# magenta/music-spectrogram-diffusion

Hardware: AMD Instinct MI355X
Metric: mel-frames/sec (higher is better)
Workload: dtype f16x3 (operands split into hi + lo half planes, 3 f16 MFMAs per product, fp32 accumulate; fp32 residual/norm/softmax/sampler); 1 GPU; base_with_context, 1000-step DDPM, CFG w=5, 1 song(s) per GPU, segment-sequential with context hand-off, 5 segments of 256 frames per GPU; precision=f16x3, precision_requested=f16x3, parallelism=song-parallel x1, mode=replicas, attention_query_planes=library default: hi + lo for Q and for the softmax weights, knobs=library defaults

## Files before the change

### include/msd_amd.h

```cpp
#ifndef MSD_AMD_H_
#define MSD_AMD_H_

#include <stdint.h>

#ifdef __cplusplus
extern "C" {
#endif

#define MSD_AMD_ABI_VERSION 7

typedef struct msd_model msd_model;

typedef enum msd_status {
  MSD_OK = 0,
  MSD_ERR_INVALID_ARGUMENT = 1,
  MSD_ERR_UNKNOWN_WEIGHT = 2,
  MSD_ERR_SHAPE_MISMATCH = 3,
  MSD_ERR_BAD_STATE = 4,
  MSD_ERR_HIP = 5,
  MSD_ERR_UNSUPPORTED = 6,
  MSD_ERR_RANGE = 7
} msd_status;

typedef enum msd_precision {
// ... 147 lines not shown
                              const float* w1_dev, const float* gamma_dev,
                              const float* film_scale_dev, const float* film_bias_dev,
                              const float* w2_dev, float* x_out_dev, float* h_out_dev,
                              int m, int k, int d, int n, void* stream);

int msd_op_geglu(const float* a_dev, const float* wi0_dev, const float* wi1_dev, float* out_dev,
                 int m, int k, int f, void* stream);

int msd_op_qkv(const float* a_dev, const float* wq_dev, const float* wk_dev, const float* wv_dev,
               float* q_out_dev, float* k_out_dev, float* v_out_dev, int m, int k, int j,
               int seg_len, void* stream);

int msd_op_final_proj(const float* x_dev, const float* gamma_dev, const float* w_dev, float* out_dev,
                      int m, int d, int n, void* stream);

int msd_op_threefry(int stage, uint64_t seed, int64_t fold, const uint32_t* bits_in_dev, float* out_dev, int64_t n,
                    void* stream);

#ifdef __cplusplus
}
#endif
#endif
```

### music-spectrogram-diffusion_amd/build_native.py

```python
from __future__ import annotations

import os
import shutil
import subprocess
import sys

HERE = os.path.dirname(os.path.abspath(__file__))
ROOT = os.path.dirname(HERE)
CSRC = os.path.join(HERE, 'csrc')
EXP = os.path.join(ROOT, 'tools', 'ubench', 'exp')
LIB = os.path.join(CSRC, 'libmsd_amd.so')
LIB_EXP = os.path.join(EXP, 'libmsd_amd_exp.so')
LIBS = {'f16': (LIB, []), 'bf16': (os.path.join(CSRC, 'libmsd_amd_bf16.so'), ['-DMSD_PLANE_BF16=1'])}
EXP_SRC = os.path.join(EXP, 'src_r04')
EXP_LIBS = {'exp': (LIB_EXP, ['-DMSD_EXPERIMENTS=1'])}
SOURCES = ['msd_api.hip']
HEADERS = ['common.h', 'phase_stamps.h', 'gemm_h16.h', 'gemm_f32.h', 'attention.h', 'elementwise.h',
           os.path.join('..', '..', 'include', 'msd_amd.h')]
EXP_HEADERS = ['chain.h', 'gemm_h16_exp.h', 'gemm_splitk_exchange.inc', 'gemm_h16_pair.h', 'gemm_h16_wide.h', 'gemm_h16_ls.h']


def _hipcc():
  for c in (os.environ.get('HIPCC'), shutil.which('hipcc'), '/opt/rocm/bin/hipcc'):
    if c and os.path.exists(c):
# ... 11 lines not shown
    deps = [os.path.join(CSRC, f) for f in SOURCES + HEADERS + [os.path.join('..', 'build_native.py')]]
  return any(os.path.getmtime(f) > t for f in deps)


def check_prefetch_registers(listing: str) -> str:
  tool = os.path.join(HERE, 'check_prefetch_regs.py')
  if not os.path.exists(tool):
    raise RuntimeError('%s is missing: the build cannot verify the prefetch registers of the library' % tool)
  out = subprocess.run([sys.executable, tool, listing], capture_output=True, text=True)
  if out.returncode != 0:
    raise RuntimeError('prefetch register check failed on %s:\n%s\n%s' % (listing, out.stdout[-3000:], out.stderr[-2000:]))
  return out.stdout.strip().split('\n')[-1]


NO_SCRATCH_KERNELS = ('sampler_step_kernel', 'threefry_normal_kernel')


def check_no_scratch(listing: str, kernels=NO_SCRATCH_KERNELS) -> str:
  import re
  text = open(listing).read()
  seen = {k: 0 for k in kernels}
  bad = []
  for m in re.finditer(r'^\s*\.amdhsa_kernel\s+(\S+)(.*?)^\s*\.end_amdhsa_kernel', text, flags=re.M | re.S):
    name, body = m.group(1), m.group(2)
    for k in kernels:
      if k in name:
        seen[k] += 1
        size = re.search(r'\.amdhsa_private_segment_fixed_size\s+(\d+)', body)
        dyn = re.search(r'\.amdhsa_uses_dynamic_stack\s+(\d+)', body)
        if size is None or int(size.group(1)) != 0 or (dyn is not None and int(dyn.group(1)) != 0):
# ... 22 lines not shown
             '-fno-gpu-rdc', '-Wno-unused-result', '-ffile-prefix-map=%s=.' % ROOT, '-ffile-prefix-map=%s=.' % tmp,
             '-cuid=msd_amd',
             '-I', src] + defs + ['-o', os.path.basename(lib)] + [os.path.join(src, s) for s in SOURCES]
      if verbose:
        print('[build_native]', ' '.join(cmd), flush=True)
      subprocess.run(cmd, check=True, cwd=tmp)
      listings = [os.path.join(tmp, f) for f in os.listdir(tmp) if f.endswith('.s') and 'gfx950' in f]
      if not listings:
        raise RuntimeError('no gfx950 device listing (*gfx950*.s, -save-temps) in %s: cannot verify the prefetch '
                           'registers; the scratch directory holds %s' % (tmp, sorted(os.listdir(tmp))))
      for l in listings:
        verdict = check_prefetch_registers(l)
        if verbose:
          print('[build_native] prefetch registers:', verdict, flush=True)
        if src == CSRC:
          verdict = check_no_scratch(l)
          if verbose:
            print('[build_native] scratch:', verdict, flush=True)
      shutil.copyfile(out, lib + '.tmp')
      os.chmod(lib + '.tmp', 0o755)
      os.replace(lib + '.tmp', lib)
  return LIB


if __name__ == '__main__':
  build(force='--force' in sys.argv, experiments='--experiments' in sys.argv)
  print(LIB)
```

### music-spectrogram-diffusion_amd/csrc/elementwise.h

```cpp
#pragma once
#include "common.h"

namespace msd {

struct NormParams {
  const float* x;
  const float* gamma;
  const float* film;
  const int* step_ptr;
  int film_slots, film_slot;
  int rows, D;
  h16_t* out[2];
  float* out_f32;
  unsigned* sat = nullptr;
  unsigned sat_tag = 1;
};

template <int OUT, int VPL>
__global__ void __launch_bounds__(256) rmsnorm_film_kernel(NormParams p) {
  const int lane = threadIdx.x & 63;
  const int row = blockIdx.x * 4 + (threadIdx.x >> 6);
  if (row >= p.rows) return;
  const float* xr = p.x + (size_t)row * p.D;
  float4 v[VPL];
// ... 183 lines not shown
  const uint32_t* rng_key = nullptr;
  const float* coef;
  int* step_ptr;
  int step_from_slot1 = 0;
  int n;
  int passes;
  float cond_wt;
  int clip_x0, ddim;
  int model_output = kOutEps;
  h16_t* z_hi;
  h16_t* z_lo;
  unsigned* sat = nullptr;
  unsigned sat_tag = 1;
};

template <int mode>
__device__ __forceinline__ void convert_model_output(const float (&c)[kCoefCount], float z, float o,
                                                     float& eps, float& x0) {
  if constexpr (mode == kOutEps) {
    eps = o;
    x0 = c[kCoefMX0Scale] * (z - o * c[kCoefMX0Eps]);
  } else if constexpr (mode == kOutX0) {
    x0 = o;
    eps = c[kCoefMEpsScale] * (z - o * c[kCoefMEpsX0]);
  } else {
    x0 = c[kCoefMAlpha] * z - c[kCoefMSigma] * o;
    eps = c[kCoefMEpsScale] * (z - x0 * c[kCoefMEpsX0]);
  }
}

template <int MODE>
__device__ __forceinline__ float sampler_update(const SamplerParams& p, const float (&c)[kCoefCount], int i, float z,
                                                float o_c, float o_u, float nz) {
  float eps, x0;
  convert_model_output<MODE>(c, z, o_c, eps, x0);
  if (p.passes == 2) {
    float eps_u, x0_u;
    convert_model_output<MODE>(c, z, o_u, eps_u, x0_u);
    eps = p.cond_wt * eps + (1.0f - p.cond_wt) * eps_u;
    x0 = c[kCoefX0Scale] * (z - eps * c[kCoefX0Eps]);
  }
  if (p.clip_x0) {
    x0 = x0 < -1.0f ? -1.0f : (x0 > 1.0f ? 1.0f : x0);
    eps = c[kCoefEpsScale] * (z - x0 * c[kCoefEpsX0]);
  }
  float zs;
  if (p.ddim) zs = c[kCoefAlphaS] * x0 + c[kCoefSigmaS] * eps;
  else zs = c[kCoefMeanZ] * z + c[kCoefMeanX0] * x0 + c[kCoefStd] * nz;
  return (i == 0) ? x0 : zs;
}

template <int MODE>
__global__ void __launch_bounds__(256) sampler_step_kernel(SamplerParams p) {
  warm_kernargs<kernarg_lines<SamplerParams>()>();
  const int i = p.step_from_slot1 ? p.step_ptr[1] : p.step_ptr[0];
  typedef uint32_t u32x4 __attribute__((ext_vector_type(4)));
  const float* noise = *p.noise_slot;
  u32x4 rk0 = reinterpret_cast<const u32x4*>(p.rng_key)[0], rk1 = reinterpret_cast<const u32x4*>(p.rng_key)[1];
  static_assert(kRngKind == 4 && kRngTfKey0 == 5 && kRngTfKey1 == 6, "rk1 = {kind, Threefry key, pad}");
  asm volatile("" : "+v"(noise), "+v"(rk0), "+v"(rk1));
  const int idx = (blockIdx.x * 256 + threadIdx.x) * 4;
  if (idx < p.n) {
    const f32x4 zz = *reinterpret_cast<const f32x4*>(p.z + idx);
    const f32x4 ec = *reinterpret_cast<const f32x4*>(p.eps + idx);
    f32x4 eu = {0.f, 0.f, 0.f, 0.f}, nz = {0.f, 0.f, 0.f, 0.f};
    if (p.passes == 2) eu = *reinterpret_cast<const f32x4*>(p.eps + p.n + idx);
    static_assert(kCoefCount == 20, "five 16-byte loads per row");
    f32x4 cr[5];
#pragma unroll
    for (int k = 0; k < 5; ++k) cr[k] = reinterpret_cast<const f32x4*>(p.coef + (size_t)i * kCoefCount)[k];
    if (!p.ddim && i != 0) {
      if (noise != nullptr) {
        nz = *reinterpret_cast<const f32x4*>(noise + (size_t)i * p.n + idx);
      } else if (rk1[0] == kRngThreefry) {
        uint32_t f0 = 0u, f1 = (uint32_t)i;
        threefry2x32(rk1[1], rk1[2], f0, f1);
        const uint32_t half = (uint32_t)p.n >> 1;
#pragma unroll
        for (int k = 0; k < 4; ++k) nz[k] = threefry_normal_at(f0, f1, (uint32_t)(idx + k), half);
      } else {
        float d[4];
        philox_normal4((uint32_t)(idx >> 2), 1u + (uint32_t)i, rk0[0], rk0[1], rk0[2], rk0[3], d);
        nz = f32x4{d[0], d[1], d[2], d[3]};
      }
    }
    float c[kCoefCount];
#pragma unroll
    for (int k = 0; k < kCoefCount; ++k) c[k] = cr[k >> 2][k & 3];
    f32x4 out;
#pragma unroll
    for (int k = 0; k < 4; ++k) out[k] = sampler_update<MODE>(p, c, i, zz[k], ec[k], eu[k], nz[k]);
    *reinterpret_cast<f32x4*>(p.z + idx) = out;
    if (p.z_hi) {
      uint32_t h[2], l[2];
      RangeCheck rc;
#pragma unroll
      for (int k = 0; k < 2; ++k) {
        rc.see(out[2 * k], out[2 * k + 1]);
        split2_h16(out[2 * k], out[2 * k + 1], h[k], l[k]);
      }
      *reinterpret_cast<uint2*>(p.z_hi + idx) = make_uint2(h[0], h[1]);
      if (p.z_lo) *reinterpret_cast<uint2*>(p.z_lo + idx) = make_uint2(l[0], l[1]);
      rc.commit(p.sat, p.sat_tag);
    }
  }
  __syncthreads();
  if (blockIdx.x == gridDim.x - 1 && threadIdx.x == 0) p.step_ptr[p.step_from_slot1 ? 0 : 1] = i - 1;
}

inline void launch_sampler_step(const SamplerParams& sp, hipStream_t s) {
  const dim3 grid((sp.n / 4 + 255) / 256), block(256);
  if (sp.model_output == kOutX0) hipLaunchKernelGGL(sampler_step_kernel<kOutX0>, grid, block, 0, s, sp);
  else if (sp.model_output == kOutV) hipLaunchKernelGGL(sampler_step_kernel<kOutV>, grid, block, 0, s, sp);
  else hipLaunchKernelGGL(sampler_step_kernel<kOutEps>, grid, block, 0, s, sp);
}

__global__ void build_g_kernel(const float* film, const float* gamma, float* g, int n_steps, int slots,
                               int slot, int D) {
  const int i = blockIdx.x * 256 + threadIdx.x;
// ... 89 lines not shown
```

### music-spectrogram-diffusion_amd/csrc/gemm_f32.h

```cpp
#pragma once
#include "common.h"

namespace msd {

struct GemmF32Params {
  const float* A;
  const float* B;
  int lda, ldb;
  int M, N, K;
};

struct EpiF32Store {
  float* out;
  int ldc;
  __device__ void operator()(int m, int n, float v) const { out[(size_t)m * ldc + n] = v; }
};
struct EpiF32Swish {
  float* out;
  int ldc;
  __device__ void operator()(int m, int n, float v) const {
    out[(size_t)m * ldc + n] = v / (1.0f + expf(-v));
  }
};
struct EpiF32StoreGated {
// ... 161 lines not shown
  for (int i = 0; i < RT; ++i)
#pragma unroll
    for (int j = 0; j < 2; ++j)
#pragma unroll
      for (int e = 0; e < 4; ++e) red[wave][i * 16 + g * 4 + e][j * 16 + r] = acc[i][j][e];
  __syncthreads();
  for (int item = threadIdx.x; item < BMR * 32; item += 64 * kFinalProjWaves) {
    const int m = item >> 5, n = item & 31;
    float v = 0.f;
#pragma unroll
    for (int w = 0; w < kFinalProjWaves; ++w) v += red[w][m][n];
    p.out[(size_t)(m0 + m) * p.N + n0 + n] = v * rstd[m];
  }
}

__global__ void scale_rows_kernel(const float* w, const float* gamma, float* wg, int K, int N) {
  const int i = blockIdx.x * 256 + threadIdx.x;
  if (i < K * N) wg[i] = gamma[i / N] * w[i];
}

template <class Epi>
inline hipError_t launch_gemm_f32(const GemmF32Params& p, const Epi& epi, hipStream_t stream) {
  const int grid = ((p.M + 63) / 64) * (p.N / 64);
  hipLaunchKernelGGL(gemm_f32_kernel<Epi>, dim3(grid), dim3(256), 0, stream, p, epi);
  return hipGetLastError();
}

}
```

### music-spectrogram-diffusion_amd/csrc/msd_api.hip

```cpp
#include <hip/hip_runtime.h>
#include <algorithm>
#include <cctype>
#include <cmath>
#include <cstdarg>
#include <cstdio>
#include <cstdlib>
#include <cstring>
#include <string>
#include <unordered_map>
#include <vector>

#include "../../include/msd_amd.h"
#include "attention.h"
#include "common.h"
#include "elementwise.h"
#include "gemm_h16.h"
#include "gemm_f32.h"

using namespace msd;

namespace {

constexpr int kHeadDim = 64;
constexpr int kDefaultQPlanes = 2, kDefaultPPlanes = 2;
// ... 930 lines not shown
    return to.bn == kNarrowTile;
  }
}

template <int NP>
EpiResidualNorm<NP, false, true> with_y2(const EpiResidualNorm<NP>& e, const Planes& y2, const float* g2, int rows) {
  EpiResidualNorm<NP, false, true> o;
  o.x = e.x; o.ldx = e.ldx; o.y[0] = e.y[0]; o.y[1] = e.y[1]; o.ssq = e.ssq; o.tiles = e.tiles;
  o.g_lo = e.g_lo; o.g_lo_stride = e.g_lo_stride; o.g_hi = e.g_hi; o.g_hi_stride = e.g_hi_stride;
  o.split_row = e.split_row; o.step_ptr = e.step_ptr; o.dup_rows = e.dup_rows;
  o.y2[0] = y2.p[0]; o.y2[1] = y2.p[NP - 1]; o.g2 = g2; o.y2_rows = rows;
  return o;
}

template <int NP>
void decoder_layers(Ctx& c, int batch, int P, bool cond0, bool dedup0 = false) {
  msd_model* m = c.m;
  const int D = m->D, J = m->J, F = m->F, T = m->T;
  const int BT = batch * T, M = P * BT;
  const int slots = 2 * m->Ld, tiles = D / kNarrowTile;
  const Planes &y = m->y, &qk = m->qk, &vts = m->vt, &ao = m->ao, &gb = m->g;
  float* const x = m->x;
  float* const ssq = m->ssq;
  float* const eps = m->eps;
  const int* const nkeys_self = m->d_nkeys_self;
  auto rowscale = [&](const float* bias, int stride) {
    RowScale r;
    r.ssq = ssq; r.tiles = tiles; r.inv_d = 1.0f / (float)D; r.bias = bias; r.bias_step_stride = stride;
    r.step_ptr = m->d_step;
    return r;
  };
// ... 123 lines not shown
      const bool fold_next = !last_layer && fold_cross_q<NP>(m, batch, P, cond0, false);
      WeightPrefetch pf_qkv = last_layer ? WeightPrefetch() : prefetch_of<NP>(m, m->dec[l + 1].self.wqkv, 3 * J + (fold_next ? nq : 0), D);
      if (fold_next) {
        if constexpr (NP == 2)
          gemm<NP, TK_TALL>(c, KC_GEMM_MLP_OUT, gb, F, w.mlp.wo, F, M, D, F, with_y2<NP>(eo, m->xg, m->dec[l + 1].ln_cross, BT), 0, &pf_qkv);
      } else {
        gemm<NP, TK_TALL>(c, KC_GEMM_MLP_OUT, gb, F, w.mlp.wo, F, M, D, F, eo, 0, &pf_qkv);
      }
    }
  }
  if (NP == 2) {
    FinalProjParams fp;
    fp.x = x; fp.wg = m->w_out_g; fp.ssq = ssq; fp.out = eps;
    fp.M = M; fp.N = m->ND; fp.K = D; fp.tiles = tiles; fp.inv_d = 1.0f / (float)D;
    c.begin(KC_FINAL_PROJ);
    hipLaunchKernelGGL(final_proj_f32_kernel<1>, dim3(m->ND / 32, M / 16), dim3(64 * kFinalProjWaves), 0, c.s, fp);
    c.end(KC_FINAL_PROJ);
  } else {
    EpiStoreF32 ef;
    ef.out = eps; ef.ldc = m->ND; ef.rsc = rowscale(nullptr, 0);
    gemm<NP, TK_NARROW>(c, KC_FINAL_PROJ, y, D, m->w_out_p, D, M, m->ND, D, ef);
  }
}

template <int NP>
void in_proj(Ctx& c, int batch, int P, bool publish_step = false, bool fold0 = false) {
  msd_model* m = c.m;
  const int BT = batch * m->T;
  EpiInProj<NP> ei;
  ei.x = m->x; ei.ldx = m->D; ei.pos = m->dec_pos; ei.T = m->T; ei.pass_rows = BT; ei.passes = P;
  ei.y[0] = m->y.p[0]; ei.y[1] = m->y.p[NP - 1]; ei.ssq = m->ssq; ei.tiles = m->D / kNarrowTile;
// ... 3 lines not shown
  WeightPrefetch pf = prefetch_of<NP>(m, m->dec[0].self.wqkv, 3 * m->J + (fold0 ? m->n_cross * m->J : 0), m->D);
  gemm<NP, TK_NARROW>(c, KC_IN_PROJ, m->zp, m->ND, m->w_in_p, m->ND, BT, m->D, m->ND, ei, 0, &pf);
}

void split_z(msd_model* m, int64_t n, hipStream_t s) {
  hipLaunchKernelGGL(split_planes_kernel, dim3((unsigned)((n + 255) / 256)), dim3(256), 0, s, m->z, m->zp.p[0],
                     m->NP == 2 ? m->zp.p[1] : (h16_t*)nullptr, n, m->d_sat, (unsigned)KC_SAMPLER + 1u);
}

template <int NP>
void enqueue_step(Ctx& c, int batch) {
  msd_model* m = c.m;
  const int P = m->passes;
  const bool dedup0 = P == 2 && m->dedup_layer0;
  in_proj<NP>(c, batch, dedup0 ? 1 : P, true, fold_cross_q<NP>(m, batch, P, true, dedup0));
  decoder_layers<NP>(c, batch, P, true, dedup0);
  SamplerParams sp;
  sp.eps = m->eps; sp.z = m->z; sp.noise_slot = m->d_noise_slot; sp.coef = m->d_coef; sp.rng_key = m->d_rng_key;
  sp.step_ptr = m->d_step; sp.n = batch * m->T * m->ND; sp.passes = P;
  sp.cond_wt = m->cfg.cfg_weight; sp.clip_x0 = m->cfg.clip_x0;
  sp.ddim = m->cfg.sampler == MSD_SAMPLER_DDIM;
  sp.model_output = m->cfg.model_output;
  sp.z_hi = m->zp.p[0];
  sp.z_lo = m->NP == 2 ? m->zp.p[1] : nullptr;
  sp.sat = m->d_sat; sp.sat_tag = (unsigned)KC_SAMPLER + 1u;
  c.begin(KC_SAMPLER);
  sp.step_from_slot1 = 1;
  launch_sampler_step(sp, c.s);
  c.end(KC_SAMPLER);
}

void set_func_attrs() {
  (void)attention_prepare<1, 3>();
  (void)attention_prepare<2, 2>();
  (void)prepare_gemms<1>();
  (void)prepare_gemms<2>();
}


}

extern "C" {
// ... 958 lines not shown
  if (hipMemcpyAsync(h.data(), f32, (size_t)M * J * sizeof(float), hipMemcpyDeviceToHost, s) != hipSuccess ||
      hipStreamSynchronize(s) != hipSuccess)
    return MSD_ERR_HIP;
  for (int m = 0; m < M; ++m) {
    const int seg = m / seg_len, key = m % seg_len, o16 = key & 15;
    const int kp = (key & ~15) + 8 * ((o16 >> 2) & 1) + (o16 & 3) + 4 * (o16 >> 3);
    for (int j = 0; j < J; ++j) vh[(size_t)m * J + j] = h[((size_t)seg * J + j) * seg_len + kp];
  }
  if (hipMemcpy(q_out_dev, qh.data(), qh.size() * sizeof(float), hipMemcpyHostToDevice) != hipSuccess ||
      hipMemcpy(k_out_dev, kh.data(), kh.size() * sizeof(float), hipMemcpyHostToDevice) != hipSuccess ||
      hipMemcpy(v_out_dev, vh.data(), vh.size() * sizeof(float), hipMemcpyHostToDevice) != hipSuccess)
    return MSD_ERR_HIP;
  return MSD_OK;
}

int msd_op_final_proj(const float* x_dev, const float* gamma_dev, const float* w_dev, float* out_dev, int M, int D,
                      int n, void* stream) {
  if (M % 64 || D % 64 || n % 32 || M <= 0 || D > 1024 || !x_dev || !gamma_dev || !w_dev || !out_dev)
    return MSD_ERR_INVALID_ARGUMENT;
  hipStream_t s = static_cast<hipStream_t>(stream);
  Scratch sc;
  const int tiles = D / kNarrowTile;
  float* x = sc.get<float>((size_t)M * D);
  float* ssq = sc.get<float>((size_t)M * tiles);
  float* wg = sc.get<float>((size_t)D * n);
  int* step = sc.get<int>(2);
  Planes za, zw;
  for (int i = 0; i < 2; ++i) { za.p[i] = sc.get<h16_t>((size_t)M * 64); zw.p[i] = sc.get<h16_t>((size_t)D * 64); }
  if (!x || !ssq || !wg || !step || !za.p[1] || !zw.p[1]) return MSD_ERR_HIP;
  if (hipMemcpyAsync(x, x_dev, (size_t)M * D * sizeof(float), hipMemcpyDeviceToDevice, s) != hipSuccess) return MSD_ERR_HIP;
  EpiResidualNorm<2> er;
  er.x = x; er.ldx = D; er.y[0] = nullptr; er.y[1] = nullptr; er.ssq = ssq; er.tiles = tiles; er.step_ptr = step;
  er.g_lo = nullptr; er.g_lo_stride = 0; er.g_hi = nullptr; er.g_hi_stride = 0; er.split_row = 0;
  hipError_t e = launch_gemm_h16_dma<2, 32, 32, 4>(gp<2>(za, 64, zw, 64, M, D, 64), er, s);
  if (e != hipSuccess) return MSD_ERR_HIP;
  hipLaunchKernelGGL(scale_rows_kernel, dim3((D * n + 255) / 256), dim3(256), 0, s, w_dev, gamma_dev, wg, D, n);
  FinalProjParams fp;
  fp.x = x; fp.wg = wg; fp.ssq = ssq; fp.out = out_dev; fp.M = M; fp.N = n; fp.K = D; fp.tiles = tiles;
  fp.inv_d = 1.0f / (float)D;
  hipLaunchKernelGGL(final_proj_f32_kernel<1>, dim3(n / 32, M / 16), dim3(64 * kFinalProjWaves), 0, s, fp);
  if (hipGetLastError() != hipSuccess) return MSD_ERR_HIP;
  return hipStreamSynchronize(s) == hipSuccess ? MSD_OK : MSD_ERR_HIP;
}

}
```

### music-spectrogram-diffusion_amd/native.py

```python
from __future__ import annotations

import ctypes
import os
from typing import Dict, List, Optional, Tuple

import numpy as np

_HERE = os.path.dirname(os.path.abspath(__file__))
LIB_PATH = os.path.join(_HERE, 'csrc', 'libmsd_amd.so')
LIB_PATHS = {'f16': LIB_PATH, 'bf16': os.path.join(_HERE, 'csrc', 'libmsd_amd_bf16.so')}

MSD_PREC_F16 = 0
MSD_PREC_F16X3 = 1
MSD_PREC_BF16 = 2
MSD_PREC_BF16X3 = 3
ABI_VERSION = 7
MSD_SAMPLER_DDPM = 0
MSD_SAMPLER_DDIM = 1
MSD_RNG_PHILOX = 0
MSD_RNG_THREEFRY = 1
RNGS = {'philox': MSD_RNG_PHILOX, 'threefry': MSD_RNG_THREEFRY}
MAX_KERNEL_CLASSES = 16

PRECISIONS = {'f16': MSD_PREC_F16, 'f16x3': MSD_PREC_F16X3, 'bf16': MSD_PREC_BF16, 'bf16x3': MSD_PREC_BF16X3}
_PLANES_OF = {MSD_PREC_F16: 'f16', MSD_PREC_F16X3: 'f16', MSD_PREC_BF16: 'bf16', MSD_PREC_BF16X3: 'bf16'}


def plane_format(precision: str) -> str:
  if precision not in PRECISIONS:
    raise ValueError('precision must be one of %s' % sorted(PRECISIONS))
  return 'bf16' if precision.startswith('bf16') else 'f16'


EXPORTED_SYMBOLS = (
    'msd_version', 'msd_device_count', 'msd_create', 'msd_destroy', 'msd_last_error',
    'msd_num_weights', 'msd_weight_info', 'msd_set_weight', 'msd_finalize_weights',
    'msd_encode', 'msd_sample', 'msd_reset_graph', 'msd_decoder_pass', 'msd_fill_normal', 'msd_get_schedule',
    'msd_debug_read', 'msd_profile_steps', 'msd_op_gemm_h16', 'msd_op_gemm_bf16', 'msd_op_gemm_f32',
    'msd_op_attention', 'msd_op_attention_qp', 'msd_op_attention_split', 'msd_op_attention_ex', 'msd_op_sampler_step', 'msd_op_residual_norm_gemm', 'msd_op_geglu',
    'msd_op_qkv', 'msd_op_final_proj', 'msd_sample_rng', 'msd_fill_normal_threefry', 'msd_op_threefry')


class NativeLibraryError(RuntimeError):
  pass


class RangeError(ArithmeticError):
  """MSD_ERR_RANGE: an activation left the range of the IEEE-half operand planes (|x| > 65504) during the call;
  its result is invalid.  The bfloat16-plane precisions ('bf16x3') have float32's exponent range."""


MSD_SCHEDULE_COSINE, MSD_SCHEDULE_LINEAR = 0, 1
MSD_OUTPUT_EPS, MSD_OUTPUT_X0, MSD_OUTPUT_V = 0, 1, 2
MSD_LOGVAR_LARGE, MSD_LOGVAR_SMALL, MSD_LOGVAR_MEDIUM = 0, 1, 2
SCHEDULES = {'cosine': MSD_SCHEDULE_COSINE, 'linear': MSD_SCHEDULE_LINEAR}
# ... 92 lines not shown
    lib.msd_op_gemm_h16.argtypes = [i32, vp, vp, vp, i32, i32, i32, vp]
  lib.msd_op_gemm_bf16.argtypes = [i32, vp, vp, vp, i32, i32, i32, vp]
  lib.msd_op_gemm_f32.argtypes = [vp, vp, vp, i32, i32, i32, vp]
  lib.msd_op_attention.argtypes = [i32, vp, vp, vp, vp, i32, i32, i32, i32, vp]
  if 'msd_op_attention_qp' in present:
    lib.msd_op_attention_qp.argtypes = [i32, i32, vp, vp, vp, vp, i32, i32, i32, i32, vp]
  if 'msd_op_attention_split' in present:
    lib.msd_op_attention_split.argtypes = [i32, i32, i32, i32, i32, vp, vp, vp, vp, i32, i32, i32, i32, vp]
  if 'msd_op_attention_ex' in present:
    lib.msd_op_attention_ex.argtypes = [i32, i32, i32, i32, i32, i32, vp, i32, vp, vp, vp, vp, i32, i32, i32, i32, vp]
  lib.msd_op_sampler_step.argtypes = [c.POINTER(MsdConfig), i32, vp, vp, vp, vp, vp, i64, vp]
  lib.msd_op_residual_norm_gemm.argtypes = [i32, vp, vp, vp, vp, vp, vp, vp, vp, vp, i32, i32, i32, i32, vp]
  lib.msd_op_geglu.argtypes = [vp, vp, vp, vp, i32, i32, i32, vp]
  lib.msd_op_qkv.argtypes = [vp, vp, vp, vp, vp, vp, vp, i32, i32, i32, i32, vp]
  lib.msd_op_final_proj.argtypes = [vp, vp, vp, vp, i32, i32, i32, vp]
  for name in present:
    fn = getattr(lib, name)
    if name not in ('msd_version', 'msd_last_error', 'msd_destroy'):
      fn.restype = i32
  _libs[planes] = lib
  return lib


_EXC = {1: ValueError, 2: KeyError, 3: ValueError, 4: RuntimeError, 5: RuntimeError,
        6: NotImplementedError, 7: RangeError}


def _check(lib, handle, rc, what):
  if rc == 0:
    return
# ... 239 lines not shown
  _op_check(lib.msd_op_geglu(_ptr(a), _ptr(wi0), _ptr(wi1), _ptr(out), m, k, wi0.shape[1], stream), 'msd_op_geglu')


def op_qkv(a, wq, wk, wv, q, k_out, v, seg_len: int, stream: int = 0):
  lib = load()
  m, k = a.shape
  _op_check(lib.msd_op_qkv(_ptr(a), _ptr(wq), _ptr(wk), _ptr(wv), _ptr(q), _ptr(k_out), _ptr(v), m, k,
                           wq.shape[1], seg_len, stream), 'msd_op_qkv')


def op_final_proj(x, gamma, w, out, stream: int = 0):
  lib = load()
  m, d = x.shape
  _op_check(lib.msd_op_final_proj(_ptr(x), _ptr(gamma), _ptr(w), _ptr(out), m, d, w.shape[1], stream),
            'msd_op_final_proj')
```

Before: 266.2 mel-frames/sec.

## Fuse final projection with DDPM sampler step in one kernel

Adds a fused kernel that computes the final RMS-normed output projection for the cond and uncond passes in the same block, then has one wave run the CFG/DDPM sampler update, split z into f16 hi/lo planes, and advance the step counter. The separate sampler launch and its global round trip of eps per diffusion step are removed on the f16x3 path (NP==2). The sampler math now uses explicit fmaf with contraction off so the two paths round the same way. The trade-off is a final-proj grid of 16x16 tiles per block instead of 32-wide tiles, and extra register pressure from holding the sampler state.

New measurement: 265.4 mel-frames/sec. About the same (-0.3%).

```diff
diff --git a/include/msd_amd.h b/include/msd_amd.h
--- a/include/msd_amd.h
+++ b/include/msd_amd.h
@@ -185,6 +185,11 @@
 int msd_op_final_proj(const float* x_dev, const float* gamma_dev, const float* w_dev, float* out_dev,
                       int m, int d, int n, void* stream);
 
+int msd_op_final_sampler(const float* x_dev, const float* gamma_dev, const float* w_dev, float* eps_out_dev,
+                         int m, int d, int n, const msd_config* cfg, int step_index, const float* z_dev,
+                         const float* noise_dev, int rng, uint64_t seed, uint64_t stream_id, float* z_out_dev,
+                         void* z_hi_out_dev, void* z_lo_out_dev, int* step_slots_out, void* stream);
+
 int msd_op_threefry(int stage, uint64_t seed, int64_t fold, const uint32_t* bits_in_dev, float* out_dev, int64_t n,
                     void* stream);
 
diff --git a/music-spectrogram-diffusion_amd/build_native.py b/music-spectrogram-diffusion_amd/build_native.py
--- a/music-spectrogram-diffusion_amd/build_native.py
+++ b/music-spectrogram-diffusion_amd/build_native.py
@@ -49,6 +49,7 @@
 
 
 NO_SCRATCH_KERNELS = ('sampler_step_kernel', 'threefry_normal_kernel')
+FUSED_TAIL_KERNELS = ('final_sampler_step_kernel',)
 
 
 def check_no_scratch(listing: str, kernels=NO_SCRATCH_KERNELS) -> str:
@@ -101,9 +102,10 @@
         if verbose:
           print('[build_native] prefetch registers:', verdict, flush=True)
         if src == CSRC:
-          verdict = check_no_scratch(l)
-          if verbose:
-            print('[build_native] scratch:', verdict, flush=True)
+          for kernels in (NO_SCRATCH_KERNELS, FUSED_TAIL_KERNELS):
+            verdict = check_no_scratch(l, kernels)
+            if verbose:
+              print('[build_native] scratch:', verdict, flush=True)
       shutil.copyfile(out, lib + '.tmp')
       os.chmod(lib + '.tmp', 0o755)
       os.replace(lib + '.tmp', lib)
diff --git a/music-spectrogram-diffusion_amd/csrc/elementwise.h b/music-spectrogram-diffusion_amd/csrc/elementwise.h
--- a/music-spectrogram-diffusion_amd/csrc/elementwise.h
+++ b/music-spectrogram-diffusion_amd/csrc/elementwise.h
@@ -221,47 +221,99 @@
   unsigned sat_tag = 1;
 };
 
-template <int mode>
+template <int mode, bool UNCOND>
 __device__ __forceinline__ void convert_model_output(const float (&c)[kCoefCount], float z, float o,
                                                      float& eps, float& x0) {
+#pragma clang fp contract(off)
   if constexpr (mode == kOutEps) {
     eps = o;
-    x0 = c[kCoefMX0Scale] * (z - o * c[kCoefMX0Eps]);
+    x0 = c[kCoefMX0Scale] * fmaf(-o, c[kCoefMX0Eps], z);
   } else if constexpr (mode == kOutX0) {
     x0 = o;
-    eps = c[kCoefMEpsScale] * (z - o * c[kCoefMEpsX0]);
+    eps = c[kCoefMEpsScale] * fmaf(-o, c[kCoefMEpsX0], z);
   } else {
-    x0 = c[kCoefMAlpha] * z - c[kCoefMSigma] * o;
-    eps = c[kCoefMEpsScale] * (z - x0 * c[kCoefMEpsX0]);
+    const float az = c[kCoefMAlpha] * z;
+    if constexpr (UNCOND) {
+      x0 = fmaf(-o, c[kCoefMSigma], az);
+    } else {
+      const float so = c[kCoefMSigma] * o;
+      x0 = az - so;
+    }
+    eps = c[kCoefMEpsScale] * fmaf(-x0, c[kCoefMEpsX0], z);
   }
 }
 
 template <int MODE>
 __device__ __forceinline__ float sampler_update(const SamplerParams& p, const float (&c)[kCoefCount], int i, float z,
                                                 float o_c, float o_u, float nz) {
+#pragma clang fp contract(off)
   float eps, x0;
-  convert_model_output<MODE>(c, z, o_c, eps, x0);
+  convert_model_output<MODE, false>(c, z, o_c, eps, x0);
   if (p.passes == 2) {
     float eps_u, x0_u;
-    convert_model_output<MODE>(c, z, o_u, eps_u, x0_u);
-    eps = p.cond_wt * eps + (1.0f - p.cond_wt) * eps_u;
-    x0 = c[kCoefX0Scale] * (z - eps * c[kCoefX0Eps]);
+    convert_model_output<MODE, true>(c, z, o_u, eps_u, x0_u);
+    const float wc = p.cond_wt * eps, wu = (1.0f - p.cond_wt) * eps_u;
+    eps = wc + wu;
+    x0 = c[kCoefX0Scale] * fmaf(-eps, c[kCoefX0Eps], z);
   }
   if (p.clip_x0) {
     x0 = x0 < -1.0f ? -1.0f : (x0 > 1.0f ? 1.0f : x0);
-    eps = c[kCoefEpsScale] * (z - x0 * c[kCoefEpsX0]);
+    eps = c[kCoefEpsScale] * fmaf(-x0, c[kCoefEpsX0], z);
   }
   float zs;
-  if (p.ddim) zs = c[kCoefAlphaS] * x0 + c[kCoefSigmaS] * eps;
-  else zs = c[kCoefMeanZ] * z + c[kCoefMeanX0] * x0 + c[kCoefStd] * nz;
+  if (p.ddim) {
+    const float ax = c[kCoefAlphaS] * x0;
+    zs = fmaf(eps, c[kCoefSigmaS], ax);
+  } else {
+    const float mz = c[kCoefMeanZ] * z, mx = c[kCoefMeanX0] * x0;
+    const float mean = mz + mx;
+    zs = fmaf(nz, c[kCoefStd], mean);
+  }
   return (i == 0) ? x0 : zs;
+}
+
+typedef uint32_t u32x4 __attribute__((ext_vector_type(4)));
+__device__ __forceinline__ f32x4 sampler_noise4(const SamplerParams& p, int i, int idx, const float* noise,
+                                                const u32x4& rk0, const u32x4& rk1) {
+  f32x4 nz = {0.f, 0.f, 0.f, 0.f};
+  if (!p.ddim && i != 0) {
+    if (noise != nullptr) {
+      nz = *reinterpret_cast<const f32x4*>(noise + (size_t)i * p.n + idx);
+    } else if (rk1[0] == kRngThreefry) {
+      uint32_t f0 = 0u, f1 = (uint32_t)i;
+      threefry2x32(rk1[1], rk1[2], f0, f1);
+      const uint32_t half = (uint32_t)p.n >> 1;
+#pragma unroll
+      for (int k = 0; k < 4; ++k) nz[k] = threefry_normal_at(f0, f1, (uint32_t)(idx + k), half);
+    } else {
+      float d[4];
+      philox_normal4((uint32_t)(idx >> 2), 1u + (uint32_t)i, rk0[0], rk0[1], rk0[2], rk0[3], d);
+      nz = f32x4{d[0], d[1], d[2], d[3]};
+    }
+  }
+  return nz;
+}
+
+__device__ __forceinline__ void sampler_store4(const SamplerParams& p, int idx, const f32x4& out) {
+  *reinterpret_cast<f32x4*>(p.z + idx) = out;
+  if (p.z_hi) {
+    uint32_t h[2], l[2];
+    RangeCheck rc;
+#pragma unroll
+    for (int k = 0; k < 2; ++k) {
+      rc.see(out[2 * k], out[2 * k + 1]);
+      split2_h16(out[2 * k], out[2 * k + 1], h[k], l[k]);
+    }
+    *reinterpret_cast<uint2*>(p.z_hi + idx) = make_uint2(h[0], h[1]);
+    if (p.z_lo) *reinterpret_cast<uint2*>(p.z_lo + idx) = make_uint2(l[0], l[1]);
+    rc.commit(p.sat, p.sat_tag);
+  }
 }
 
 template <int MODE>
 __global__ void __launch_bounds__(256) sampler_step_kernel(SamplerParams p) {
   warm_kernargs<kernarg_lines<SamplerParams>()>();
   const int i = p.step_from_slot1 ? p.step_ptr[1] : p.step_ptr[0];
-  typedef uint32_t u32x4 __attribute__((ext_vector_type(4)));
   const float* noise = *p.noise_slot;
   u32x4 rk0 = reinterpret_cast<const u32x4*>(p.rng_key)[0], rk1 = reinterpret_cast<const u32x4*>(p.rng_key)[1];
   static_assert(kRngKind == 4 && kRngTfKey0 == 5 && kRngTfKey1 == 6, "rk1 = {kind, Threefry key, pad}");
@@ -270,46 +322,20 @@
   if (idx < p.n) {
     const f32x4 zz = *reinterpret_cast<const f32x4*>(p.z + idx);
     const f32x4 ec = *reinterpret_cast<const f32x4*>(p.eps + idx);
-    f32x4 eu = {0.f, 0.f, 0.f, 0.f}, nz = {0.f, 0.f, 0.f, 0.f};
+    f32x4 eu = {0.f, 0.f, 0.f, 0.f};
     if (p.passes == 2) eu = *reinterpret_cast<const f32x4*>(p.eps + p.n + idx);
     static_assert(kCoefCount == 20, "five 16-byte loads per row");
     f32x4 cr[5];
 #pragma unroll
     for (int k = 0; k < 5; ++k) cr[k] = reinterpret_cast<const f32x4*>(p.coef + (size_t)i * kCoefCount)[k];
-    if (!p.ddim && i != 0) {
-      if (noise != nullptr) {
-        nz = *reinterpret_cast<const f32x4*>(noise + (size_t)i * p.n + idx);
-      } else if (rk1[0] == kRngThreefry) {
-        uint32_t f0 = 0u, f1 = (uint32_t)i;
-        threefry2x32(rk1[1], rk1[2], f0, f1);
-        const uint32_t half = (uint32_t)p.n >> 1;
-#pragma unroll
-        for (int k = 0; k < 4; ++k) nz[k] = threefry_normal_at(f0, f1, (uint32_t)(idx + k), half);
-      } else {
-        float d[4];
-        philox_normal4((uint32_t)(idx >> 2), 1u + (uint32_t)i, rk0[0], rk0[1], rk0[2], rk0[3], d);
-        nz = f32x4{d[0], d[1], d[2], d[3]};
-      }
-    }
+    const f32x4 nz = sampler_noise4(p, i, idx, noise, rk0, rk1);
     float c[kCoefCount];
 #pragma unroll
     for (int k = 0; k < kCoefCount; ++k) c[k] = cr[k >> 2][k & 3];
     f32x4 out;
 #pragma unroll
     for (int k = 0; k < 4; ++k) out[k] = sampler_update<MODE>(p, c, i, zz[k], ec[k], eu[k], nz[k]);
-    *reinterpret_cast<f32x4*>(p.z + idx) = out;
-    if (p.z_hi) {
-      uint32_t h[2], l[2];
-      RangeCheck rc;
-#pragma unroll
-      for (int k = 0; k < 2; ++k) {
-        rc.see(out[2 * k], out[2 * k + 1]);
-        split2_h16(out[2 * k], out[2 * k + 1], h[k], l[k]);
-      }
-      *reinterpret_cast<uint2*>(p.z_hi + idx) = make_uint2(h[0], h[1]);
-      if (p.z_lo) *reinterpret_cast<uint2*>(p.z_lo + idx) = make_uint2(l[0], l[1]);
-      rc.commit(p.sat, p.sat_tag);
-    }
+    sampler_store4(p, idx, out);
   }
   __syncthreads();
   if (blockIdx.x == gridDim.x - 1 && threadIdx.x == 0) p.step_ptr[p.step_from_slot1 ? 0 : 1] = i - 1;
diff --git a/music-spectrogram-diffusion_amd/csrc/gemm_f32.h b/music-spectrogram-diffusion_amd/csrc/gemm_f32.h
--- a/music-spectrogram-diffusion_amd/csrc/gemm_f32.h
+++ b/music-spectrogram-diffusion_amd/csrc/gemm_f32.h
@@ -1,5 +1,6 @@
 #pragma once
 #include "common.h"
+#include "elementwise.h"
 
 namespace msd {
 
@@ -199,6 +200,135 @@
   }
 }
 
+struct FinalSamplerParams {
+  FinalProjParams fp;
+  SamplerParams sp;
+  int rows;
+};
+
+template <int MODE>
+__global__ void __launch_bounds__(64 * kFinalProjWaves) final_sampler_step_kernel(FinalSamplerParams q) {
+#pragma clang fp contract(off)
+  warm_kernargs<kernarg_lines<FinalSamplerParams>()>();
+  const FinalProjParams& p = q.fp;
+  const SamplerParams& sp = q.sp;
+  constexpr int kSamplerWave = kFinalProjWaves - 1;
+  __shared__ __attribute__((aligned(16))) float red[kFinalProjWaves][32][17];
+  __shared__ __attribute__((aligned(16))) float eps_s[2][16][16];
+  __shared__ float rstd[32];
+  const int lane = threadIdx.x & 63;
+  const int wave = __builtin_amdgcn_readfirstlane(threadIdx.x >> 6);
+  const int m0 = blockIdx.y * 16, n0 = blockIdx.x * 16;
+  const int pass_off = sp.passes == 2 ? q.rows : 0;
+  const int g = lane >> 4, r = lane & 15;
+  const int idx = (m0 + (lane >> 2)) * p.N + n0 + (lane & 3) * 4;
+  int i = 0;
+  const float* noise = nullptr;
+  u32x4 rk0 = {0u, 0u, 0u, 0u}, rk1 = {0u, 0u, 0u, 0u};
+  f32x4 zz = {0.f, 0.f, 0.f, 0.f}, nz = {0.f, 0.f, 0.f, 0.f};
+  f32x4 cr[5];
+#pragma unroll
+  for (int k = 0; k < 5; ++k) cr[k] = f32x4{0.f, 0.f, 0.f, 0.f};
+  if (wave == kSamplerWave) {
+    i = sp.step_from_slot1 ? sp.step_ptr[1] : sp.step_ptr[0];
+    noise = *sp.noise_slot;
+    rk0 = reinterpret_cast<const u32x4*>(sp.rng_key)[0];
+    rk1 = reinterpret_cast<const u32x4*>(sp.rng_key)[1];
+    asm volatile("" : "+v"(noise), "+v"(rk0), "+v"(rk1));
+    zz = *reinterpret_cast<const f32x4*>(sp.z + idx);
+#pragma unroll
+    for (int k = 0; k < 5; ++k) cr[k] = reinterpret_cast<const f32x4*>(sp.coef + (size_t)i * kCoefCount)[k];
+  }
+  float ss = 0.f;
+  float sv[8];
+  if (wave < 2) {
+    const int row = lane & 15, part = lane >> 4;
+    const int per = (p.tiles + 3) >> 2;
+    const float* s = p.ssq + (size_t)(m0 + wave * pass_off + row) * p.tiles;
+#pragma unroll
+    for (int k = 0; k < 8; ++k) {
+      const int t = part * per + k;
+      sv[k] = s[(k < per && t < p.tiles) ? t : 0];
+    }
+  }
+  f32x4 acc[2];
+  acc[0] = f32x4{0.f, 0.f, 0.f, 0.f};
+  acc[1] = f32x4{0.f, 0.f, 0.f, 0.f};
+  const float* xa = p.x + (size_t)(m0 + r) * p.K + 4 * g;
+  const float* wb = p.wg + (size_t)(4 * g) * p.N + n0 + r;
+  constexpr int U = 6;
+  for (int kb = wave * 16; kb < p.K; kb += 16 * kFinalProjWaves * U) {
+    float4 a[U][2];
+    float b[U][4];
+#pragma unroll
+    for (int u = 0; u < U; ++u) {
+      const int k0 = kb + u * 16 * kFinalProjWaves;
+      const int kk = k0 < p.K ? k0 : kb;
+#pragma unroll
+      for (int t = 0; t < 2; ++t) a[u][t] = *reinterpret_cast<const float4*>(xa + (size_t)(t * pass_off) * p.K + kk);
+#pragma unroll
+      for (int c = 0; c < 4; ++c) b[u][c] = wb[(size_t)(kk + c) * p.N];
+    }
+    if (wave == kSamplerWave && kb == wave * 16) nz = sampler_noise4(sp, i, idx, noise, rk0, rk1);
+#pragma unroll
+    for (int u = 0; u < U; ++u) {
+      if (kb + u * 16 * kFinalProjWaves < p.K) {
+#pragma unroll
+        for (int c = 0; c < 4; ++c) {
+#pragma unroll
+          for (int t = 0; t < 2; ++t) {
+            const float av = c == 0 ? a[u][t].x : (c == 1 ? a[u][t].y : (c == 2 ? a[u][t].z : a[u][t].w));
+            acc[t] = __builtin_amdgcn_mfma_f32_16x16x4f32(av, b[u][c], acc[t], 0, 0, 0);
+          }
+        }
+      }
+    }
+  }
+  if (wave < 2) {
+    const int part = lane >> 4, per = (p.tiles + 3) >> 2;
+#pragma unroll
+    for (int k = 0; k < 8; ++k) ss += (k < per && part * per + k < p.tiles) ? sv[k] : 0.f;
+    ss += __shfl_xor(ss, 16, 64);
+    ss += __shfl_xor(ss, 32, 64);
+    if (lane < 16) rstd[wave * 16 + lane] = 1.0f / sqrtf(fmaf(ss, p.inv_d, 1e-6f));
+  }
+#pragma unroll
+  for (int t = 0; t < 2; ++t)
+#pragma unroll
+    for (int e = 0; e < 4; ++e) red[wave][t * 16 + g * 4 + e][r] = acc[t][e];
+  __syncthreads();
+  {
+    const int t = threadIdx.x >> 8, m = (threadIdx.x >> 4) & 15, n = threadIdx.x & 15;
+    float v = 0.f;
+#pragma unroll
+    for (int w = 0; w < kFinalProjWaves; ++w) v += red[w][t * 16 + m][n];
+    const float e = v * rstd[t * 16 + m];
+    if (t == 0 || sp.passes == 2) p.out[(size_t)(t * q.rows + m0 + m) * p.N + n0 + n] = e;
+    eps_s[t][m][n] = e;
+  }
+  __syncthreads();
+  if (wave == kSamplerWave) {
+    const f32x4 ec = *reinterpret_cast<const f32x4*>(&eps_s[0][lane >> 2][(lane & 3) * 4]);
+    const f32x4 eu = *reinterpret_cast<const f32x4*>(&eps_s[1][lane >> 2][(lane & 3) * 4]);
+    float c[kCoefCount];
+#pragma unroll
+    for (int k = 0; k < kCoefCount; ++k) c[k] = cr[k >> 2][k & 3];
+    f32x4 out;
+#pragma unroll
+    for (int k = 0; k < 4; ++k) out[k] = sampler_update<MODE>(sp, c, i, zz[k], ec[k], eu[k], nz[k]);
+    sampler_store4(sp, idx, out);
+    if (blockIdx.x == gridDim.x - 1 && blockIdx.y == gridDim.y - 1 && lane == 0)
+      sp.step_ptr[sp.step_from_slot1 ? 0 : 1] = i - 1;
+  }
+}
+
+inline void launch_final_sampler_step(const FinalSamplerParams& q, hipStream_t s) {
+  const dim3 grid(q.fp.N / 16, q.rows / 16), block(64 * kFinalProjWaves);
+  if (q.sp.model_output == kOutX0) hipLaunchKernelGGL(final_sampler_step_kernel<kOutX0>, grid, block, 0, s, q);
+  else if (q.sp.model_output == kOutV) hipLaunchKernelGGL(final_sampler_step_kernel<kOutV>, grid, block, 0, s, q);
+  else hipLaunchKernelGGL(final_sampler_step_kernel<kOutEps>, grid, block, 0, s, q);
+}
+
 __global__ void scale_rows_kernel(const float* w, const float* gamma, float* wg, int K, int N) {
   const int i = blockIdx.x * 256 + threadIdx.x;
   if (i < K * N) wg[i] = gamma[i / N] * w[i];
diff --git a/music-spectrogram-diffusion_amd/csrc/msd_api.hip b/music-spectrogram-diffusion_amd/csrc/msd_api.hip
--- a/music-spectrogram-diffusion_amd/csrc/msd_api.hip
+++ b/music-spectrogram-diffusion_amd/csrc/msd_api.hip
@@ -968,7 +968,7 @@
 }
 
 template <int NP>
-void decoder_layers(Ctx& c, int batch, int P, bool cond0, bool dedup0 = false) {
+void decoder_layers(Ctx& c, int batch, int P, bool cond0, bool dedup0 = false, const SamplerParams* sampler = nullptr) {
   msd_model* m = c.m;
   const int D = m->D, J = m->J, F = m->F, T = m->T;
   const int BT = batch * T, M = P * BT;
@@ -1122,7 +1122,13 @@
     fp.x = x; fp.wg = m->w_out_g; fp.ssq = ssq; fp.out = eps;
     fp.M = M; fp.N = m->ND; fp.K = D; fp.tiles = tiles; fp.inv_d = 1.0f / (float)D;
     c.begin(KC_FINAL_PROJ);
-    hipLaunchKernelGGL(final_proj_f32_kernel<1>, dim3(m->ND / 32, M / 16), dim3(64 * kFinalProjWaves), 0, c.s, fp);
+    if (sampler) {
+      FinalSamplerParams q;
+      q.fp = fp; q.sp = *sampler; q.rows = BT;
+      launch_final_sampler_step(q, c.s);
+    } else {
+      hipLaunchKernelGGL(final_proj_f32_kernel<1>, dim3(m->ND / 32, M / 16), dim3(64 * kFinalProjWaves), 0, c.s, fp);
+    }
     c.end(KC_FINAL_PROJ);
   } else {
     EpiStoreF32 ef;
@@ -1156,7 +1162,6 @@
   const int P = m->passes;
   const bool dedup0 = P == 2 && m->dedup_layer0;
   in_proj<NP>(c, batch, dedup0 ? 1 : P, true, fold_cross_q<NP>(m, batch, P, true, dedup0));
-  decoder_layers<NP>(c, batch, P, true, dedup0);
   SamplerParams sp;
   sp.eps = m->eps; sp.z = m->z; sp.noise_slot = m->d_noise_slot; sp.coef = m->d_coef; sp.rng_key = m->d_rng_key;
   sp.step_ptr = m->d_step; sp.n = batch * m->T * m->ND; sp.passes = P;
@@ -1166,8 +1171,13 @@
   sp.z_hi = m->zp.p[0];
   sp.z_lo = m->NP == 2 ? m->zp.p[1] : nullptr;
   sp.sat = m->d_sat; sp.sat_tag = (unsigned)KC_SAMPLER + 1u;
+  sp.step_from_slot1 = 1;
+  if (NP == 2) {
+    decoder_layers<NP>(c, batch, P, true, dedup0, &sp);
+    return;
+  }
+  decoder_layers<NP>(c, batch, P, true, dedup0);
   c.begin(KC_SAMPLER);
-  sp.step_from_slot1 = 1;
   launch_sampler_step(sp, c.s);
   c.end(KC_SAMPLER);
 }
@@ -2156,33 +2166,97 @@
   return MSD_OK;
 }
 
+extern "C++" {
+namespace {
+bool final_proj_operands(Scratch& sc, const float* x_dev, const float* gamma_dev, const float* w_dev, int M, int D, int n,
+                         hipStream_t s, FinalProjParams* fp) {
+  const int tiles = D / kNarrowTile, Mp = (M + 63) / 64 * 64;
+  float* x = sc.get<float>((size_t)Mp * D);
+  float* ssq = sc.get<float>((size_t)Mp * tiles);
+  float* wg = sc.get<float>((size_t)D * n);
+  int* step = sc.get<int>(2);
+  Planes za, zw;
+  for (int i = 0; i < 2; ++i) { za.p[i] = sc.get<h16_t>((size_t)Mp * 64); zw.p[i] = sc.get<h16_t>((size_t)D * 64); }
+  if (!x || !ssq || !wg || !step || !za.p[1] || !zw.p[1]) return false;
+  if (hipMemcpyAsync(x, x_dev, (size_t)M * D * sizeof(float), hipMemcpyDeviceToDevice, s) != hipSuccess) return false;
+  EpiResidualNorm<2> er;
+  er.x = x; er.ldx = D; er.y[0] = nullptr; er.y[1] = nullptr; er.ssq = ssq; er.tiles = tiles; er.step_ptr = step;
+  er.g_lo = nullptr; er.g_lo_stride = 0; er.g_hi = nullptr; er.g_hi_stride = 0; er.split_row = 0;
+  if (launch_gemm_h16_dma<2, 32, 32, 4>(gp<2>(za, 64, zw, 64, Mp, D, 64), er, s) != hipSuccess) return false;
+  hipLaunchKernelGGL(scale_rows_kernel, dim3((D * n + 255) / 256), dim3(256), 0, s, w_dev, gamma_dev, wg, D, n);
+  fp->x = x; fp->wg = wg; fp->ssq = ssq; fp->out = nullptr; fp->M = M; fp->N = n; fp->K = D; fp->tiles = tiles;
+  fp->inv_d = 1.0f / (float)D;
+  return true;
+}
+}
+}
+
 int msd_op_final_proj(const float* x_dev, const float* gamma_dev, const float* w_dev, float* out_dev, int M, int D,
                       int n, void* stream) {
-  if (M % 64 || D % 64 || n % 32 || M <= 0 || D > 1024 || !x_dev || !gamma_dev || !w_dev || !out_dev)
+  if (M % 16 || D % 64 || n % 32 || M <= 0 || D > 1024 || !x_dev || !gamma_dev || !w_dev || !out_dev)
     return MSD_ERR_INVALID_ARGUMENT;
   hipStream_t s = static_cast<hipStream_t>(stream);
   Scratch sc;
-  const int tiles = D / kNarrowTile;
-  float* x = sc.get<float>((size_t)M * D);
-  float* ssq = sc.get<float>((size_t)M * tiles);
-  float* wg = sc.get<float>((size_t)D * n);
-  int* step = sc.get<int>(2);
-  Planes za, zw;
-  for (int i = 0; i < 2; ++i) { za.p[i] = sc.get<h16_t>((size_t)M * 64); zw.p[i] = sc.get<h16_t>((size_t)D * 64); }
-  if (!x || !ssq || !wg || !step || !za.p[1] || !zw.p[1]) return MSD_ERR_HIP;
-  if (hipMemcpyAsync(x, x_dev, (size_t)M * D * sizeof(float), hipMemcpyDeviceToDevice, s) != hipSuccess) return MSD_ERR_HIP;
-  EpiResidualNorm<2> er;
-  er.x = x; er.ldx = D; er.y[0] = nullptr; er.y[1] = nullptr; er.ssq = ssq; er.tiles = tiles; er.step_ptr = step;
-  er.g_lo = nullptr; er.g_lo_stride = 0; er.g_hi = nullptr; er.g_hi_stride = 0; er.split_row = 0;
-  hipError_t e = launch_gemm_h16_dma<2, 32, 32, 4>(gp<2>(za, 64, zw, 64, M, D, 64), er, s);
-  if (e != hipSuccess) return MSD_ERR_HIP;
-  hipLaunchKernelGGL(scale_rows_kernel, dim3((D * n + 255) / 256), dim3(256), 0, s, w_dev, gamma_dev, wg, D, n);
   FinalProjParams fp;
-  fp.x = x; fp.wg = wg; fp.ssq = ssq; fp.out = out_dev; fp.M = M; fp.N = n; fp.K = D; fp.tiles = tiles;
-  fp.inv_d = 1.0f / (float)D;
+  if (!final_proj_operands(sc, x_dev, gamma_dev, w_dev, M, D, n, s, &fp)) return MSD_ERR_HIP;
+  fp.out = out_dev;
   hipLaunchKernelGGL(final_proj_f32_kernel<1>, dim3(n / 32, M / 16), dim3(64 * kFinalProjWaves), 0, s, fp);
   if (hipGetLastError() != hipSuccess) return MSD_ERR_HIP;
   return hipStreamSynchronize(s) == hipSuccess ? MSD_OK : MSD_ERR_HIP;
 }
 
-}
+int msd_op_final_sampler(const float* x_dev, const float* gamma_dev, const float* w_dev, float* eps_out_dev, int M, int D,
+                         int n, const msd_config* cfg, int step_index, const float* z_dev, const float* noise_dev,
+                         int rng, uint64_t seed, uint64_t stream_id, float* z_out_dev, void* z_hi_out_dev,
+                         void* z_lo_out_dev, int* step_slots_out, void* stream) {
+  if (!cfg || cfg->struct_size != (int32_t)sizeof(msd_config) || M <= 0 || D % 64 || D > 1024 || n % 32 || n <= 0 ||
+      !x_dev || !gamma_dev || !w_dev || !eps_out_dev || !z_dev || !z_out_dev || step_index < 0 ||
+      step_index >= cfg->num_steps || (rng != MSD_RNG_PHILOX && rng != MSD_RNG_THREEFRY) || (z_lo_out_dev && !z_hi_out_dev))
+    return MSD_ERR_INVALID_ARGUMENT;
+  const int passes = cfg->cfg_weight != 1.0f ? 2 : 1;
+  if (M % (16 * passes)) return MSD_ERR_INVALID_ARGUMENT;
+  const int rows = M / passes;
+  const int64_t nz = (int64_t)rows * n;
+  std::vector<float> coef_rows;
+  std::string why;
+  if (!build_coef_rows(*cfg, &coef_rows, &why)) return MSD_ERR_INVALID_ARGUMENT;
+  hipStream_t s = static_cast<hipStream_t>(stream);
+  Scratch sc;
+  FinalSamplerParams q;
+  if (!final_proj_operands(sc, x_dev, gamma_dev, w_dev, M, D, n, s, &q.fp)) return MSD_ERR_HIP;
+  q.fp.out = eps_out_dev;
+  q.rows = rows;
+  float* coef = sc.get<float>(coef_rows.size());
+  const float** slot = sc.get<const float*>(1);
+  int* step = sc.get<int>(2);
+  uint32_t* key = sc.get<uint32_t>(kRngWords);
+  unsigned* sat = sc.get<unsigned>(1);
+  if (!coef || !slot || !step || !key || !sat) return MSD_ERR_HIP;
+  const float* base = noise_dev ? noise_dev - (size_t)step_index * nz : nullptr;
+  const int st[2] = {step_index, step_index};
+  uint32_t hkey[kRngWords];
+  fill_rng_key(hkey, rng, seed, stream_id);
+  if (hipMemcpyAsync(coef, coef_rows.data(), coef_rows.size() * sizeof(float), hipMemcpyHostToDevice, s) != hipSuccess ||
+      hipMemcpyAsync(z_out_dev, z_dev, nz * sizeof(float), hipMemcpyDeviceToDevice, s) != hipSuccess ||
+      hipMemcpyAsync(slot, &base, sizeof(base), hipMemcpyHostToDevice, s) != hipSuccess ||
+      hipMemcpyAsync(step, st, sizeof(st), hipMemcpyHostToDevice, s) != hipSuccess ||
+      hipMemcpyAsync(key, hkey, sizeof(hkey), hipMemcpyHostToDevice, s) != hipSuccess ||
+      hipStreamSynchronize(s) != hipSuccess)
+    return MSD_ERR_HIP;
+  SamplerParams& sp = q.sp;
+  sp.eps = eps_out_dev; sp.z = z_out_dev; sp.noise_slot = slot; sp.coef = coef; sp.step_ptr = step; sp.rng_key = key;
+  sp.n = (int)nz; sp.passes = passes; sp.cond_wt = cfg->cfg_weight; sp.clip_x0 = cfg->clip_x0;
+  sp.ddim = cfg->sampler == MSD_SAMPLER_DDIM; sp.model_output = cfg->model_output;
+  sp.z_hi = static_cast<h16_t*>(z_hi_out_dev); sp.z_lo = static_cast<h16_t*>(z_lo_out_dev);
+  sp.sat = sat; sp.sat_tag = 1u; sp.step_from_slot1 = 1;
+  launch_final_sampler_step(q, s);
+  if (hipGetLastError() != hipSuccess) return MSD_ERR_HIP;
+  int st_out[2] = {0, 0};
+  if (hipMemcpyAsync(st_out, step, sizeof(st_out), hipMemcpyDeviceToHost, s) != hipSuccess ||
+      hipStreamSynchronize(s) != hipSuccess)
+    return MSD_ERR_HIP;
+  if (step_slots_out) { step_slots_out[0] = st_out[0]; step_slots_out[1] = st_out[1]; }
+  return MSD_OK;
+}
+
+}
diff --git a/music-spectrogram-diffusion_amd/native.py b/music-spectrogram-diffusion_amd/native.py
--- a/music-spectrogram-diffusion_amd/native.py
+++ b/music-spectrogram-diffusion_amd/native.py
@@ -38,7 +38,8 @@
     'msd_encode', 'msd_sample', 'msd_reset_graph', 'msd_decoder_pass', 'msd_fill_normal', 'msd_get_schedule',
     'msd_debug_read', 'msd_profile_steps', 'msd_op_gemm_h16', 'msd_op_gemm_bf16', 'msd_op_gemm_f32',
     'msd_op_attention', 'msd_op_attention_qp', 'msd_op_attention_split', 'msd_op_attention_ex', 'msd_op_sampler_step', 'msd_op_residual_norm_gemm', 'msd_op_geglu',
-    'msd_op_qkv', 'msd_op_final_proj', 'msd_sample_rng', 'msd_fill_normal_threefry', 'msd_op_threefry')
+    'msd_op_qkv', 'msd_op_final_proj', 'msd_sample_rng', 'msd_fill_normal_threefry', 'msd_op_threefry',
+    'msd_op_final_sampler')
 
 
 class NativeLibraryError(RuntimeError):
@@ -161,6 +162,9 @@
   lib.msd_op_geglu.argtypes = [vp, vp, vp, vp, i32, i32, i32, vp]
   lib.msd_op_qkv.argtypes = [vp, vp, vp, vp, vp, vp, vp, i32, i32, i32, i32, vp]
   lib.msd_op_final_proj.argtypes = [vp, vp, vp, vp, i32, i32, i32, vp]
+  if 'msd_op_final_sampler' in present:
+    lib.msd_op_final_sampler.argtypes = [vp, vp, vp, vp, i32, i32, i32, c.POINTER(MsdConfig), i32, vp, vp, i32, u64, u64,
+                                         vp, vp, vp, c.POINTER(i32), vp]
   for name in present:
     fn = getattr(lib, name)
     if name not in ('msd_version', 'msd_last_error', 'msd_destroy'):
@@ -430,3 +434,14 @@
   m, d = x.shape
   _op_check(lib.msd_op_final_proj(_ptr(x), _ptr(gamma), _ptr(w), _ptr(out), m, d, w.shape[1], stream),
             'msd_op_final_proj')
+
+
+def op_final_sampler(cfg: MsdConfig, step_index: int, x, gamma, w, z, noise, eps_out, z_out, z_hi=None, z_lo=None,
+                     rng: str = 'philox', seed: int = 0, stream_id: int = 0, stream: int = 0):
+  lib = load()
+  m, d = x.shape
+  slots = (ctypes.c_int * 2)()
+  _op_check(lib.msd_op_final_sampler(_ptr(x), _ptr(gamma), _ptr(w), _ptr(eps_out), m, d, w.shape[1], ctypes.byref(cfg),
+                                     step_index, _ptr(z), _ptr(noise), RNGS[rng], seed, stream_id, _ptr(z_out),
+                                     _ptr(z_hi), _ptr(z_lo), slots, stream), 'msd_op_final_sampler')
+  return slots[0], slots[1]
```
